# intel/neural-speed

Measured on NVIDIA H100. Metric: decode tokens/s + prefill tok/s Llama-2-7B Q4_0 @1 GPU; % HBM roofline, higher is better.
Workload: dtype int8xint4->f32 (q8_0 x q4_0)

## Files before the change

### neural_speed_b200/csrc/gemm_tc.cu

```cuda
#include <cuda.h>

#include "nsb.cuh"

namespace {

constexpr int BLOCK_N = 128;
constexpr int BLOCK_K = 64;
constexpr int WG_K = 16;
constexpr int DEQ_TILE = BLOCK_N * BLOCK_K * 2;
constexpr int kConsumerThreads = 256, kDequantThreads = 128, kThreads = kConsumerThreads + kDequantThreads + 32;

struct GemmParams {
  const uint8_t* rows;
  int wfmt, f4kind;
  int pitch, sc_off, zp_off, stype, asym, group, ngroups;
  int n, k, kpad, m;
  float* dst;
  int ldo;
  const float* bias;
  int bias_bcast;
  const float* residual;
  int kb_per_split;
  int dbg;
};

__device__ __forceinline__ uint32_t smem_u32(const void* p) { return (uint32_t)__cvta_generic_to_shared(p); }
__device__ __forceinline__ void mbar_init(uint64_t* bar, int count) {
  asm volatile("mbarrier.init.shared::cta.b64 [%0], %1;" ::"r"(smem_u32(bar)), "r"(count) : "memory");
}
__device__ __forceinline__ void mbar_expect_tx(uint64_t* bar, uint32_t bytes) {
  asm volatile("mbarrier.arrive.expect_tx.shared::cta.b64 _, [%0], %1;" ::"r"(smem_u32(bar)), "r"(bytes) : "memory");
}
__device__ __forceinline__ void mbar_arrive(uint64_t* bar) {
  asm volatile("mbarrier.arrive.shared::cta.b64 _, [%0];" ::"r"(smem_u32(bar)) : "memory");
}
__device__ __forceinline__ void mbar_wait(uint64_t* bar, uint32_t parity) {
  uint32_t ok;
  do {
    asm volatile(
        "{\n"
        ".reg .pred p;\n"
        "mbarrier.try_wait.parity.shared::cta.b64 p, [%1], %2;\n"
        "selp.u32 %0, 1, 0, p;\n"
        "}\n"
        : "=r"(ok)
        : "r"(smem_u32(bar)), "r"(parity)
        : "memory");
  } while (!ok);
}
__device__ __forceinline__ void tma_load_2d(void* dst, const CUtensorMap* map, int x, int y, uint64_t* bar) {
  asm volatile(
      "cp.async.bulk.tensor.2d.shared::cluster.global.tile.mbarrier::complete_tx::bytes [%0], [%1, {%2, %3}], [%4];" ::"r"(
          smem_u32(dst)),
      "l"(map), "r"(x), "r"(y), "r"(smem_u32(bar))
      : "memory");
}
__device__ __forceinline__ uint64_t make_desc_sw128(uint32_t smem_addr) {
  return (uint64_t)((smem_addr & 0x3FFFFu) >> 4) | (1ull << 16) | (64ull << 32) | (1ull << 62);
}
__device__ __forceinline__ void wgmma_fence() { asm volatile("wgmma.fence.sync.aligned;" ::: "memory"); }
__device__ __forceinline__ void wgmma_commit() { asm volatile("wgmma.commit_group.sync.aligned;" ::: "memory"); }
template <int N>
__device__ __forceinline__ void wgmma_wait() {
  asm volatile("wgmma.wait_group.sync.aligned %0;" ::"n"(N) : "memory");
}
__device__ __forceinline__ void wgmma_m64n32k16(float (&d)[16], uint64_t adesc, uint64_t bdesc) {
  asm volatile(
      "{\n.reg .pred p;\nsetp.ne.b32 p, %18, 0;\n"
      "wgmma.mma_async.sync.aligned.m64n32k16.f32.bf16.bf16 {"
      "%0, %1, %2, %3, %4, %5, %6, %7, %8, %9, %10, %11, %12, %13, %14, %15"
      "}, %16, %17, p, 1, 1, 0, 0;\n}\n"
      : "+f"(d[0]), "+f"(d[1]), "+f"(d[2]), "+f"(d[3]), "+f"(d[4]), "+f"(d[5]), "+f"(d[6]), "+f"(d[7]),
        "+f"(d[8]), "+f"(d[9]), "+f"(d[10]), "+f"(d[11]), "+f"(d[12]), "+f"(d[13]), "+f"(d[14]), "+f"(d[15])
      : "l"(adesc), "l"(bdesc), "r"(1));
}
__device__ __forceinline__ void wgmma_m64n64k16(float (&d)[32], uint64_t adesc, uint64_t bdesc) {
  asm volatile(
      "{\n.reg .pred p;\nsetp.ne.b32 p, %34, 0;\n"
      "wgmma.mma_async.sync.aligned.m64n64k16.f32.bf16.bf16 {"
      "%0, %1, %2, %3, %4, %5, %6, %7, %8, %9, %10, %11, %12, %13, %14, %15, "
      "%16, %17, %18, %19, %20, %21, %22, %23, %24, %25, %26, %27, %28, %29, %30, %31"
      "}, %32, %33, p, 1, 1, 0, 0;\n}\n"
      : "+f"(d[0]), "+f"(d[1]), "+f"(d[2]), "+f"(d[3]), "+f"(d[4]), "+f"(d[5]), "+f"(d[6]), "+f"(d[7]),
        "+f"(d[8]), "+f"(d[9]), "+f"(d[10]), "+f"(d[11]), "+f"(d[12]), "+f"(d[13]), "+f"(d[14]), "+f"(d[15]),
        "+f"(d[16]), "+f"(d[17]), "+f"(d[18]), "+f"(d[19]), "+f"(d[20]), "+f"(d[21]), "+f"(d[22]), "+f"(d[23]),
        "+f"(d[24]), "+f"(d[25]), "+f"(d[26]), "+f"(d[27]), "+f"(d[28]), "+f"(d[29]), "+f"(d[30]), "+f"(d[31])
      : "l"(adesc), "l"(bdesc), "r"(1));
}
__device__ __forceinline__ void wgmma_m64n128k16(float (&d)[64], uint64_t adesc, uint64_t bdesc) {
  asm volatile(
      "{\n.reg .pred p;\nsetp.ne.b32 p, %66, 0;\n"
      "wgmma.mma_async.sync.aligned.m64n128k16.f32.bf16.bf16 {"
      "%0, %1, %2, %3, %4, %5, %6, %7, %8, %9, %10, %11, %12, %13, %14, %15, "
      "%16, %17, %18, %19, %20, %21, %22, %23, %24, %25, %26, %27, %28, %29, %30, %31, "
      "%32, %33, %34, %35, %36, %37, %38, %39, %40, %41, %42, %43, %44, %45, %46, %47, "
      "%48, %49, %50, %51, %52, %53, %54, %55, %56, %57, %58, %59, %60, %61, %62, %63"
      "}, %64, %65, p, 1, 1, 0, 0;\n}\n"
      : "+f"(d[0]), "+f"(d[1]), "+f"(d[2]), "+f"(d[3]), "+f"(d[4]), "+f"(d[5]), "+f"(d[6]), "+f"(d[7]),
        "+f"(d[8]), "+f"(d[9]), "+f"(d[10]), "+f"(d[11]), "+f"(d[12]), "+f"(d[13]), "+f"(d[14]), "+f"(d[15]),
        "+f"(d[16]), "+f"(d[17]), "+f"(d[18]), "+f"(d[19]), "+f"(d[20]), "+f"(d[21]), "+f"(d[22]), "+f"(d[23]),
        "+f"(d[24]), "+f"(d[25]), "+f"(d[26]), "+f"(d[27]), "+f"(d[28]), "+f"(d[29]), "+f"(d[30]), "+f"(d[31]),
        "+f"(d[32]), "+f"(d[33]), "+f"(d[34]), "+f"(d[35]), "+f"(d[36]), "+f"(d[37]), "+f"(d[38]), "+f"(d[39]),
        "+f"(d[40]), "+f"(d[41]), "+f"(d[42]), "+f"(d[43]), "+f"(d[44]), "+f"(d[45]), "+f"(d[46]), "+f"(d[47]),
        "+f"(d[48]), "+f"(d[49]), "+f"(d[50]), "+f"(d[51]), "+f"(d[52]), "+f"(d[53]), "+f"(d[54]), "+f"(d[55]),
        "+f"(d[56]), "+f"(d[57]), "+f"(d[58]), "+f"(d[59]), "+f"(d[60]), "+f"(d[61]), "+f"(d[62]), "+f"(d[63])
      : "l"(adesc), "l"(bdesc), "r"(1));
}

template <int T>
__device__ __forceinline__ void wgmma_k16(float (&d)[T / 2], uint64_t adesc, uint64_t bdesc) {
  if constexpr (T == 32) wgmma_m64n32k16(d, adesc, bdesc);
  else if constexpr (T == 64) wgmma_m64n64k16(d, adesc, bdesc);
  else wgmma_m64n128k16(d, adesc, bdesc);
}

template <int T, bool W8 = false>
struct Smem {
  static constexpr int SP = 6;
  static constexpr int SD = 3;
  static constexpr int SA = T >= 128 ? 4 : 6;
  static constexpr int ROW_BYTES = W8 ? BLOCK_K : BLOCK_K / 2;
  static constexpr int PACKED_STAGE = BLOCK_N * ROW_BYTES;
  static constexpr int DEQ_STAGE = DEQ_TILE;
  static constexpr int ACT_STAGE = T * BLOCK_K * 2;
  static constexpr int off_deq = 0;
  static constexpr int off_act = off_deq + SD * DEQ_STAGE;
  static constexpr int off_packed = off_act + SA * ACT_STAGE;
  static constexpr int off_bar = off_packed + SP * PACKED_STAGE;
  static constexpr int num_bars = 2 * SP + 2 * SA + 2 * SD;
  static constexpr int total = off_bar + num_bars * 8 + 1024;
};

template <int T, bool W8>
__global__ void __launch_bounds__(kThreads, 1)
    gemm_w4_tc_kernel(const __grid_constant__ CUtensorMap tmap_w, const __grid_constant__ CUtensorMap tmap_a, const GemmParams P) {
  using L = Smem<T, W8>;
  constexpr int ROW_BYTES = L::ROW_BYTES;
  constexpr int SA = L::SA, SP = L::SP, SD = L::SD, PACKED_STAGE = L::PACKED_STAGE, DEQ_STAGE = L::DEQ_STAGE;
  extern __shared__ unsigned char smem_raw[];
  unsigned char* smem = smem_raw + ((1024 - (smem_u32(smem_raw) & 1023)) & 1023);
  unsigned char* deq = smem + L::off_deq;
  unsigned char* act = smem + L::off_act;
  unsigned char* packed = smem + L::off_packed;
  uint64_t* bars = reinterpret_cast<uint64_t*>(smem + L::off_bar);
  uint64_t* p_full = bars;
  uint64_t* p_empty = p_full + SP;
  uint64_t* a_full = p_empty + SP;
  uint64_t* a_empty = a_full + SA;
  uint64_t* d_full = a_empty + SA;
  uint64_t* d_empty = d_full + SD;

  const int warp = threadIdx.x >> 5, lane = threadIdx.x & 31;
  const int n0 = blockIdx.x * BLOCK_N;
  const int t0 = blockIdx.y * T;
  const int total_kb = (P.kpad + BLOCK_K - 1) / BLOCK_K;
  const int kb0 = blockIdx.z * P.kb_per_split;
  const int num_kb = (total_kb - kb0 < P.kb_per_split) ? total_kb - kb0 : P.kb_per_split;

  __shared__ float nf4_lut[16];
  if (threadIdx.x >= 32 && threadIdx.x < 48) nf4_lut[threadIdx.x - 32] = NS_F4_LUT[P.f4kind][threadIdx.x - 32];
  pdl_launch_dependents();
  if (threadIdx.x == 0) {
    for (int i = 0; i < SP; ++i) {
      mbar_init(&p_full[i], 1);
      mbar_init(&p_empty[i], kDequantThreads / 32);
    }
    for (int i = 0; i < SA; ++i) {
      mbar_init(&a_full[i], 1);
      mbar_init(&a_empty[i], kConsumerThreads / 128);
    }
    for (int i = 0; i < SD; ++i) {
      mbar_init(&d_full[i], kDequantThreads / 32);
      mbar_init(&d_empty[i], kConsumerThreads / 128);
    }
    asm volatile("fence.mbarrier_init.release.cluster;" ::: "memory");
  }
  if (warp == 12 && lane == 0) {
    asm volatile("prefetch.tensormap [%0];" ::"l"(&tmap_w) : "memory");
    asm volatile("prefetch.tensormap [%0];" ::"l"(&tmap_a) : "memory");
  }
  __syncthreads();

  if (warp == 12) {
    if (lane == 0) {
      const int pre = num_kb < SP ? num_kb : SP;
      for (int kb = 0; kb < pre; ++kb) {
        mbar_expect_tx(&p_full[kb], PACKED_STAGE);
        tma_load_2d(packed + kb * PACKED_STAGE, &tmap_w, (kb0 + kb) * ROW_BYTES, n0, &p_full[kb]);
      }
      pdl_wait();
      for (int kb = 0; kb < num_kb; ++kb) {
        const int sa = kb % SA;
        if (kb >= SA) mbar_wait(&a_empty[sa], ((kb / SA) - 1) & 1);
        mbar_expect_tx(&a_full[sa], L::ACT_STAGE);
        tma_load_2d(act + sa * L::ACT_STAGE, &tmap_a, (kb0 + kb) * BLOCK_K, t0, &a_full[sa]);
        const int kp = kb + SP;
        if (kp < num_kb) {
          const int sp = kp % SP;
          mbar_wait(&p_empty[sp], ((kp / SP) - 1) & 1);
          mbar_expect_tx(&p_full[sp], PACKED_STAGE);
          tma_load_2d(packed + sp * PACKED_STAGE, &tmap_w, (kb0 + kp) * ROW_BYTES, n0, &p_full[sp]);
        }
      }
    }
  } else if (warp >= 8) {
    const int r = threadIdx.x - kConsumerThreads;
    int grow = n0 + r;
    if (grow >= P.n) grow = P.n - 1;
    const uint8_t* rowp = P.rows + (size_t)grow * P.pitch;
    const int swz = r & 7;
    for (int kb = 0; kb < num_kb; ++kb) {
      const int sp = kb % SP, sd = kb % SD;
      int g0 = ((kb0 + kb) * BLOCK_K) / P.group, g1 = ((kb0 + kb) * BLOCK_K + 32) / P.group;
      if (g0 >= P.ngroups) g0 = P.ngroups - 1;
      if (g1 >= P.ngroups) g1 = P.ngroups - 1;
      const float sc0 = ns_scale_at(rowp + P.sc_off, P.stype, g0);
      const float sc1 = (g1 == g0) ? sc0 : ns_scale_at(rowp + P.sc_off, P.stype, g1);
      float of0 = W8 ? 0.f : 136.f, of1 = of0;
      if (P.asym) {
        of0 += (float)(int)(signed char)rowp[P.zp_off + g0];
        of1 += (float)(int)(signed char)rowp[P.zp_off + g1];
      }
      const __nv_bfloat162 s2[2] = {__float2bfloat162_rn(sc0), __float2bfloat162_rn(sc1)};
      const __nv_bfloat162 o2[2] = {__float2bfloat162_rn(of0), __float2bfloat162_rn(of1)};

      mbar_wait(&p_full[sp], (kb / SP) & 1);
      const uint4* pk = reinterpret_cast<const uint4*>(packed + sp * PACKED_STAGE + r * ROW_BYTES);
      uint32_t words[W8 ? 16 : 8];
#pragma unroll
      for (int i = 0; i < (W8 ? 4 : 2); ++i) {
        const uint4 qv = pk[i];
        words[4 * i] = qv.x, words[4 * i + 1] = qv.y, words[4 * i + 2] = qv.z, words[4 * i + 3] = qv.w;
      }
      __syncwarp();
      if (lane == 0) mbar_arrive(&p_empty[sp]);
      if (kb >= SD) mbar_wait(&d_empty[sd], ((kb / SD) - 1) & 1);
      unsigned char* drow_base = deq + sd * DEQ_STAGE + (r >> 3) * 1024 + swz * 128;
      if (!(P.dbg & 1))
#pragma unroll
      for (int c = 0; c < 8; ++c) {
        const int h = c >> 2;
        uint32_t o[4];
        if (W8) {
#pragma unroll
          for (int j = 0; j < 4; ++j) {
            const uint32_t wsrc = words[2 * c + (j >> 1)];
            const int b0 = (int)(signed char)((wsrc >> (16 * (j & 1))) & 0xffu), b1 = (int)(signed char)((wsrc >> (16 * (j & 1) + 8)) & 0xffu);
            __nv_bfloat162 v = __floats2bfloat162_rn((float)b0, (float)b1);
            v = __hmul2(__hsub2(v, o2[h]), s2[h]);
            o[j] = *reinterpret_cast<uint32_t*>(&v);
          }
        } else if (P.wfmt == NS_W_NF4) {
#pragma unroll
          for (int j = 0; j < 4; ++j) {
            const float l0 = nf4_lut[(words[c] >> (4 * j)) & 0xFu], l1 = nf4_lut[(words[c] >> (4 * j + 16)) & 0xFu];
            __nv_bfloat162 v = __hmul2(__floats2bfloat162_rn(l0, l1), s2[h]);
            o[j] = *reinterpret_cast<uint32_t*>(&v);
          }
        } else {
#pragma unroll
          for (int j = 0; j < 4; ++j) {
            uint32_t t = ((words[c] >> (4 * j)) & 0x000F000Fu) | 0x43004300u;
            __nv_bfloat162 v = *reinterpret_cast<__nv_bfloat162*>(&t);
            v = __hmul2(__hsub2(v, o2[h]), s2[h]);
            o[j] = *reinterpret_cast<uint32_t*>(&v);
          }
        }
        *reinterpret_cast<uint4*>(drow_base + ((c ^ swz) << 4)) = make_uint4(o[0], o[1], o[2], o[3]);
      }
      asm volatile("fence.proxy.async.shared::cta;" ::: "memory");
      __syncwarp();
      if (lane == 0) mbar_arrive(&d_full[sd]);
    }
  } else {
    const int g = warp >> 2;
    const bool leader = (threadIdx.x & 127) == 0;
    float acc[T / 2];
#pragma unroll
    for (int i = 0; i < T / 2; ++i) acc[i] = 0.f;
    for (int kb = 0; kb < num_kb; ++kb) {
      const int sd = kb % SD, sa = kb % SA;
      mbar_wait(&d_full[sd], (kb / SD) & 1);
      mbar_wait(&a_full[sa], (kb / SA) & 1);
      const uint32_t a_addr = smem_u32(deq + sd * DEQ_STAGE) + g * (64 * BLOCK_K * 2);
      const uint32_t b_addr = smem_u32(act + sa * L::ACT_STAGE);
      if (!(P.dbg & 2)) {
        wgmma_fence();
#pragma unroll
        for (int k4 = 0; k4 < BLOCK_K / WG_K; ++k4)
          wgmma_k16<T>(acc, make_desc_sw128(a_addr + k4 * WG_K * 2), make_desc_sw128(b_addr + k4 * WG_K * 2));
        wgmma_commit();
      }
      wgmma_wait<1>();
      if (kb > 0 && leader) {
        mbar_arrive(&d_empty[(kb - 1) % SD]);
        mbar_arrive(&a_empty[(kb - 1) % SA]);
      }
    }
    wgmma_wait<0>();
    pdl_wait();
    if (!(P.dbg & 4)) {
#pragma unroll
      for (int h = 0; h < 2; ++h) {
        const int nrow = n0 + g * 64 + (warp & 3) * 16 + (lane >> 2) + 8 * h;
        if (nrow >= P.n) continue;
        const float bcast_bias = (P.bias && P.bias_bcast) ? P.bias[nrow] : 0.f;
#pragma unroll
        for (int j = 0; j < T / 8; ++j)
#pragma unroll
          for (int e = 0; e < 2; ++e) {
            const int t = t0 + 8 * j + 2 * (lane & 3) + e;
            if (t < P.m) {
              const size_t o = (size_t)t * P.ldo + nrow;
              float x = acc[4 * j + 2 * h + e];
              if (blockIdx.z == 0) {
                x += bcast_bias;
                if (P.bias && !P.bias_bcast) x += P.bias[o];
                if (P.residual) x += P.residual[o];
              }
              if (gridDim.z > 1) atomicAdd(P.dst + o, x);
              else P.dst[o] = x;
            }
          }
      }
    }
  }
}

__global__ void __launch_bounds__(256) act_to_bf16_kernel(const float* __restrict__ A, int lda, int M, int K, int kpad,
                                                          const int* __restrict__ shuffle, __nv_bfloat16* __restrict__ out) {
  pdl_launch_dependents();
  pdl_wait();
  const size_t idx = (size_t)blockIdx.x * blockDim.x + threadIdx.x;
  const size_t total = (size_t)M * (kpad >> 1);
  if (idx >= total) return;
  const int m = (int)(idx / (kpad >> 1)), k = (int)(idx - (size_t)m * (kpad >> 1)) * 2;
  float a = 0.f, b = 0.f;
  if (k < K) a = A[(size_t)m * lda + (shuffle ? shuffle[k] : k)];
  if (k + 1 < K) b = A[(size_t)m * lda + (shuffle ? shuffle[k + 1] : k + 1)];
  reinterpret_cast<__nv_bfloat162*>(out)[idx] = __floats2bfloat162_rn(a, b);
}
__global__ void __launch_bounds__(256) act_to_bf16_v8_kernel(const float* __restrict__ A, int lda, int M, int K,
                                                             __nv_bfloat16* __restrict__ out) {
  pdl_launch_dependents();
  pdl_wait();
  const int k8 = K >> 3;
  const size_t total = (size_t)M * k8;
  for (size_t idx = (size_t)blockIdx.x * blockDim.x + threadIdx.x; idx < total; idx += (size_t)gridDim.x * blockDim.x) {
    const int m = (int)(idx / k8), c = (int)(idx - (size_t)m * k8);
    const float4* src = (const float4*)(A + (size_t)m * lda) + 2 * c;
    const float4 x = src[0], y = src[1];
    __nv_bfloat162 p0 = __floats2bfloat162_rn(x.x, x.y), p1 = __floats2bfloat162_rn(x.z, x.w);
    __nv_bfloat162 p2 = __floats2bfloat162_rn(y.x, y.y), p3 = __floats2bfloat162_rn(y.z, y.w);
    uint4 o;
    o.x = *(uint32_t*)&p0, o.y = *(uint32_t*)&p1, o.z = *(uint32_t*)&p2, o.w = *(uint32_t*)&p3;
    ((uint4*)out)[idx] = o;
  }
}

typedef CUresult (*EncodeTiledFn)(CUtensorMap*, CUtensorMapDataType, cuuint32_t, void*, const cuuint64_t*, const cuuint64_t*,
                                  const cuuint32_t*, const cuuint32_t*, CUtensorMapInterleave, CUtensorMapSwizzle,
                                  CUtensorMapL2promotion, CUtensorMapFloatOOBfill);
EncodeTiledFn get_encode() {
  static EncodeTiledFn fn = nullptr;
  if (!fn) {
    void* p = nullptr;
    cudaDriverEntryPointQueryResult qres;
    if (cudaGetDriverEntryPoint("cuTensorMapEncodeTiled", &p, cudaEnableDefault, &qres) == cudaSuccess &&
        qres == cudaDriverEntryPointSuccess)
      fn = (EncodeTiledFn)p;
  }
  return fn;
}

template <int T, bool W8>
int launch_t(const CUtensorMap& mw, const CUtensorMap& ma, const GemmParams& P, cudaStream_t st) {
  using L = Smem<T, W8>;
  auto kern = gemm_w4_tc_kernel<T, W8>;
  static bool attr_set = false;
  if (!attr_set) {
    NS_CUDA_TRY(cudaFuncSetAttribute(kern, cudaFuncAttributeMaxDynamicSharedMemorySize, L::total));
    attr_set = true;
  }
  dim3 grid((P.n + BLOCK_N - 1) / BLOCK_N, (P.m + T - 1) / T);
  GemmParams Q = P;
  const int total_kb = (P.kpad + BLOCK_K - 1) / BLOCK_K;
  int splits = 1;
  const int tiles = (int)(grid.x * grid.y);
  static const int env_splits = getenv("NS_TC_SPLITS") ? atoi(getenv("NS_TC_SPLITS")) : 0;
  if (3 * tiles < 2 * ns_num_sms() && P.residual != P.dst && P.bias != P.dst) {
    splits = ns_num_sms() / tiles;
    if (splits > total_kb / 8) splits = total_kb / 8;
    if (splits > 16) splits = 16;
    if (splits < 1) splits = 1;
  }
  if (env_splits > 0) splits = env_splits;
  Q.kb_per_split = (total_kb + splits - 1) / splits;
  splits = (total_kb + Q.kb_per_split - 1) / Q.kb_per_split;
  grid.z = (unsigned)splits;
  if (splits > 1) NS_CUDA_TRY(cudaMemset2DAsync(P.dst, (size_t)P.ldo * 4, 0, (size_t)P.n * 4, (size_t)P.m, st));
  NS_CUDA_TRY(ns_launch_pdl(kern, grid, dim3(kThreads), (size_t)L::total, st, mw, ma, Q));
  ns_count_launch();
  return NS_OK;
}

}

size_t ns_gemm_tc_workspace_bytes(int m, int kpad) { return ns_round_up((size_t)m * kpad * 2, 256); }

bool ns_gemm_tc_supported(const ns_weight* w) {
  return (w->wfmt == NS_W_S4 || w->wfmt == NS_W_NF4 || w->wfmt == NS_W_S8) && (w->group % 32 == 0 || w->group == w->k);
}

int ns_launch_act_bf16(const ns_weight* w, const float* act, int lda, int m, void* ws, cudaStream_t st) {
  if (!w->shuffle && w->k == w->kpad && (w->k & 7) == 0 && (lda & 3) == 0 && ((uintptr_t)act & 15) == 0) {
    const size_t total8 = (size_t)m * (w->k >> 3);
    size_t blocks = (total8 + 255) / 256;
    if (blocks > (size_t)ns_num_sms() * 16) blocks = (size_t)ns_num_sms() * 16;
    NS_CUDA_TRY(ns_launch_pdl(act_to_bf16_v8_kernel, dim3((unsigned)blocks), dim3(256), 0, st, act, lda, m, w->k, (__nv_bfloat16*)ws));
    ns_count_launch();
    return NS_OK;
  }
  const size_t total = (size_t)m * (w->kpad >> 1);
  NS_CUDA_TRY(ns_launch_pdl(act_to_bf16_kernel, dim3((unsigned)((total + 255) / 256)), dim3(256), 0, st, act, lda, m, w->k,
                            w->kpad, (const int*)w->shuffle, (__nv_bfloat16*)ws));
  ns_count_launch();
  return NS_OK;
}

template <bool V4>
__global__ void __launch_bounds__(256) silu_mul_kernel(const float* __restrict__ g, const float* __restrict__ u,
// ... 90 lines not shown
  }
  const __nv_bfloat16* abf = (const __nv_bfloat16*)ws;
  const int T = m <= 32 ? 32 : (m <= 64 ? 64 : 128);
  const bool w8 = w->wfmt == NS_W_S8;
  CUtensorMap mw, ma;
  {
    cuuint64_t dims[2] = {(cuuint64_t)w->q_bytes, (cuuint64_t)w->n};
    cuuint64_t strides[1] = {(cuuint64_t)w->pitch};
    cuuint32_t box[2] = {(cuuint32_t)(w8 ? BLOCK_K : BLOCK_K / 2), (cuuint32_t)BLOCK_N};
    cuuint32_t es[2] = {1, 1};
    CUresult r = enc(&mw, CU_TENSOR_MAP_DATA_TYPE_UINT8, 2, (void*)w->rows, dims, strides, box, es, CU_TENSOR_MAP_INTERLEAVE_NONE,
                     CU_TENSOR_MAP_SWIZZLE_NONE, CU_TENSOR_MAP_L2_PROMOTION_L2_128B, CU_TENSOR_MAP_FLOAT_OOB_FILL_NONE);
    if (r != CUDA_SUCCESS) {
      ns_set_error("cuTensorMapEncodeTiled(weights) failed: %d", (int)r);
      return NS_E_CUDA;
    }
  }
  {
    cuuint64_t dims[2] = {(cuuint64_t)w->kpad, (cuuint64_t)m};
    cuuint64_t strides[1] = {(cuuint64_t)w->kpad * 2};
    cuuint32_t box[2] = {BLOCK_K, (cuuint32_t)T};
    cuuint32_t es[2] = {1, 1};
    CUresult r = enc(&ma, CU_TENSOR_MAP_DATA_TYPE_BFLOAT16, 2, (void*)abf, dims, strides, box, es, CU_TENSOR_MAP_INTERLEAVE_NONE,
                     CU_TENSOR_MAP_SWIZZLE_128B, CU_TENSOR_MAP_L2_PROMOTION_L2_128B, CU_TENSOR_MAP_FLOAT_OOB_FILL_NONE);
    if (r != CUDA_SUCCESS) {
      ns_set_error("cuTensorMapEncodeTiled(activations) failed: %d", (int)r);
      return NS_E_CUDA;
    }
  }
  GemmParams P;
  P.rows = w->rows;
  P.wfmt = w->wfmt;
  P.f4kind = w->f4kind;
  P.pitch = w->pitch;
  P.sc_off = w->sc_off;
  P.zp_off = w->zp_off;
  P.stype = w->stype;
  P.asym = w->asym;
  P.group = w->group;
  P.ngroups = w->ngroups;
  P.n = w->n;
  P.k = w->k;
  P.kpad = w->kpad;
  P.m = m;
  P.dst = dst;
  P.ldo = ldo;
  P.bias = bias;
  P.bias_bcast = bias_bcast;
  P.residual = residual;
  static const int dbg = getenv("NS_TC_DEBUG") ? atoi(getenv("NS_TC_DEBUG")) : 0;
  P.dbg = dbg;
  if (w8) {
    switch (T) {
      case 32: return launch_t<32, true>(mw, ma, P, st);
      case 64: return launch_t<64, true>(mw, ma, P, st);
      default: return launch_t<128, true>(mw, ma, P, st);
    }
  }
  switch (T) {
    case 32: return launch_t<32, false>(mw, ma, P, st);
    case 64: return launch_t<64, false>(mw, ma, P, st);
    default: return launch_t<128, false>(mw, ma, P, st);
  }
}
```

### neural_speed_b200/csrc/gemv_ring_impl.cuh

```cuda
#pragma once
#include "act_quant.cuh"

namespace {

constexpr int kConsumers = 7;
constexpr int kThreads = (kConsumers + 1) * 32;

__device__ __forceinline__ uint32_t smem_u32(const void* p) { return (uint32_t)__cvta_generic_to_shared(p); }
__device__ __forceinline__ void mbar_init(uint32_t bar, int count) {
  asm volatile("mbarrier.init.shared::cta.b64 [%0], %1;" ::"r"(bar), "r"(count) : "memory");
}
__device__ __forceinline__ void mbar_expect_tx(uint32_t bar, uint32_t bytes) {
  asm volatile("mbarrier.arrive.expect_tx.shared::cta.b64 _, [%0], %1;" ::"r"(bar), "r"(bytes) : "memory");
}
__device__ __forceinline__ void mbar_arrive(uint32_t bar) {
  asm volatile("mbarrier.arrive.shared::cta.b64 _, [%0];" ::"r"(bar) : "memory");
}
__device__ __forceinline__ void mbar_wait(uint32_t bar, uint32_t parity) {
  uint32_t ok;
  do {
    asm volatile(
        "{\n"
        ".reg .pred p;\n"
        "mbarrier.try_wait.parity.shared::cta.b64 p, [%1], %2;\n"
// ... 432 lines not shown
            const float g = acc[0][m], up = acc[ROWS - 1][m];
            const float sg = P.eltop == NS_ELT_GELU ? ns_gelu(g) : ns_silu(g);
            if (P.aux) P.aux[(size_t)m * P.ldo + ps.out0] = sg;
            P.dst[(size_t)m * P.ldo + ps.out0] = sg * up;
          }
        }
      } else {
#pragma unroll
        for (int r = 0; r < ROWS; ++r) {
          if (r == 1 && !ps.valid1) continue;
          const long long out = r ? ps.out1 : ps.out0;
#pragma unroll
          for (int m = 0; m < M; ++m) {
            if (m < P.m) {
              const size_t o = (size_t)m * P.ldo + out;
              float v = acc[r][m];
              if (P.bias) v += P.bias_bcast ? P.bias[out] : P.bias[o];
              if (P.eltop == NS_ELT_GELU) v = ns_gelu(v);
              if (P.residual) v += P.residual[o];
              P.dst[o] = v;
            }
          }
        }
      }
    }
  }
}

struct RingPlan {
  int rows, stages, active, ctas;
  size_t budget;
  double score;
};

static RingPlan plan_ring(const GemvParams& P, size_t act_region, bool wide) {
  static const int env_budget = getenv("NS_RING_BUDGET_KB") ? atoi(getenv("NS_RING_BUDGET_KB")) : 0;
  static const int env_rows = getenv("NS_RING_ROWS") ? atoi(getenv("NS_RING_ROWS")) : 0;
  const size_t budgets[2] = {(size_t)(env_budget > 0 ? env_budget : 113) * 1024, 200 * 1024};
  RingPlan best = {0, 0, 0, 0, 0, -1.0};
  for (int rows = 2; rows >= 1; --rows) {
    if (rows == 1 && P.mode == NS_GEMV_GATE_UP_SILU) continue;
    if (env_rows && rows != env_rows && !(env_rows == 1 && P.mode == NS_GEMV_GATE_UP_SILU)) continue;
    const int stage_bytes = rows * P.pitch;
    for (int i = 0; i < 2; ++i) {
      if (wide && i == 0) continue;
      const int kc = (wide && i == 1) ? 2 * kConsumers : kConsumers;
      int raw = 0;
      if (budgets[i] > act_region + 64) raw = (int)((budgets[i] - act_region - 64) / (stage_bytes + 16));
      if (raw > (wide ? 56 : 32)) raw = wide ? 56 : 32;
      const int ac = raw < kc ? raw : kc;
      if (ac < 1) continue;
      const int st = raw - raw % ac;
      const int ctas = i == 0 ? 2 : 1;
      const double score = ctas * ac * (rows == 2 ? 1.1 : 1.0) + 0.001 * st;
      if (score > best.score) best = RingPlan{rows, st, ac, ctas, budgets[i], score};
    }
  }
  return best;
}

template <int AMODE, int M, bool ASYM, int STYPE, int ROWS, bool NORM, int NC = kConsumers>
int launch_rows(const GemvParams& P, const RingPlan& plan, size_t act_region, int act_row, int red_off, cudaStream_t st) {
  auto kern = gemv_ring_kernel<AMODE, M, ASYM, STYPE, ROWS, NORM, NC>;
  constexpr int threads = (NC + (NC > kConsumers ? 2 : 1)) * 32;
  static bool attr_set = false;
  if (!attr_set) {
    NS_CUDA_TRY(cudaFuncSetAttribute(kern, cudaFuncAttributeMaxDynamicSharedMemorySize, 200 * 1024));
    attr_set = true;
  }
  const int stage_bytes = ROWS * P.pitch;
  const size_t smem = act_region + (size_t)plan.stages * stage_bytes + (size_t)plan.stages * 16;
  static const int env_cps = getenv("NS_RING_CPS") ? atoi(getenv("NS_RING_CPS")) : 0;
  const int ctas_per_sm = plan.ctas == 1 ? 1 : (env_cps > 0 ? env_cps : 2);
  RingCfg R;
  R.ring_off = (int)act_region;
  R.stages = plan.stages;
  R.active = plan.active;
  R.act_row = act_row;
  R.red_off = red_off;
  if (ROWS == 2) {
    R.units = P.npairs;
  } else {
    long long rows = 0;
    for (int i = 0; i < P.nw; ++i) rows += P.n[i];
    R.units = (int)rows;
  }
  R.cpg_magic = P.cpg > 1 ? (uint32_t)((0x100000000ull + (uint64_t)P.cpg - 1) / (uint64_t)P.cpg) : 0u;
  int grid = ns_num_sms() * ctas_per_sm;
  if (grid > R.units) grid = R.units;
  if (grid < 1) grid = 1;
  static const bool dbg = getenv("NS_RING_DEBUG") != nullptr;
  if (dbg)
    fprintf(stderr, "gemv_ring: k=%d pitch=%d rows/stage=%d stages=%d active=%d smem=%zu ctas/sm=%d\n", P.k, P.pitch, ROWS, plan.stages,
            plan.active, smem, ctas_per_sm);
  NS_CUDA_TRY(ns_launch_pdl(kern, dim3(grid), dim3(threads), smem, st, P, R));
  ns_count_launch();
  return NS_OK;
}

}
```

Before: 646.0.

## Dequantize weights in consumer registers and feed wgmma A from registers

Restructures the prefill tensor-core GEMM. The dedicated dequant warpgroup and the dequantized shared-memory tile are removed. Consumer warps now read packed int4/int8 weights from shared memory, dequantize them in registers, and issue register-sourced wgmma with BLOCK_N raised to 256. Producer warps prefetch per-stage scales and offsets, setmaxnreg rebalances registers, and the epilogue stages output through shared memory for coalesced stores. Separately, the GEMV ring planner adds a wave-balance factor to its score, and a prefill A/B benchmark script is added. Risks include register pressure in consumers and dequant ALU work now sitting on the MMA critical path.

```diff
diff --git a/neural_speed_b200/csrc/gemm_tc.cu b/neural_speed_b200/csrc/gemm_tc.cu
--- a/neural_speed_b200/csrc/gemm_tc.cu
+++ b/neural_speed_b200/csrc/gemm_tc.cu
@@ -4,11 +4,12 @@
 
 namespace {
 
-constexpr int BLOCK_N = 128;
+constexpr int BLOCK_N = 256;
 constexpr int BLOCK_K = 64;
 constexpr int WG_K = 16;
-constexpr int DEQ_TILE = BLOCK_N * BLOCK_K * 2;
-constexpr int kConsumerThreads = 256, kDequantThreads = 128, kThreads = kConsumerThreads + kDequantThreads + 32;
+constexpr int kConsumerThreads = 256, kThreads = kConsumerThreads + 128;
+constexpr int kScaleThreads = 64;
+constexpr int kProducerRegs = 56, kConsumerRegs = 224;
 
 struct GemmParams {
   const uint8_t* rows;
@@ -64,38 +65,38 @@
 __device__ __forceinline__ void wgmma_wait() {
   asm volatile("wgmma.wait_group.sync.aligned %0;" ::"n"(N) : "memory");
 }
-__device__ __forceinline__ void wgmma_m64n32k16(float (&d)[16], uint64_t adesc, uint64_t bdesc) {
+__device__ __forceinline__ void wgmma_m64n32k16(float (&d)[16], const uint32_t (&a)[4], uint64_t bdesc) {
   asm volatile(
-      "{\n.reg .pred p;\nsetp.ne.b32 p, %18, 0;\n"
+      "{\n.reg .pred p;\nsetp.ne.b32 p, %21, 0;\n"
       "wgmma.mma_async.sync.aligned.m64n32k16.f32.bf16.bf16 {"
       "%0, %1, %2, %3, %4, %5, %6, %7, %8, %9, %10, %11, %12, %13, %14, %15"
-      "}, %16, %17, p, 1, 1, 0, 0;\n}\n"
+      "}, {%16, %17, %18, %19}, %20, p, 1, 1, 0;\n}\n"
       : "+f"(d[0]), "+f"(d[1]), "+f"(d[2]), "+f"(d[3]), "+f"(d[4]), "+f"(d[5]), "+f"(d[6]), "+f"(d[7]),
         "+f"(d[8]), "+f"(d[9]), "+f"(d[10]), "+f"(d[11]), "+f"(d[12]), "+f"(d[13]), "+f"(d[14]), "+f"(d[15])
-      : "l"(adesc), "l"(bdesc), "r"(1));
-}
-__device__ __forceinline__ void wgmma_m64n64k16(float (&d)[32], uint64_t adesc, uint64_t bdesc) {
+      : "r"(a[0]), "r"(a[1]), "r"(a[2]), "r"(a[3]), "l"(bdesc), "r"(1));
+}
+__device__ __forceinline__ void wgmma_m64n64k16(float (&d)[32], const uint32_t (&a)[4], uint64_t bdesc) {
   asm volatile(
-      "{\n.reg .pred p;\nsetp.ne.b32 p, %34, 0;\n"
+      "{\n.reg .pred p;\nsetp.ne.b32 p, %37, 0;\n"
       "wgmma.mma_async.sync.aligned.m64n64k16.f32.bf16.bf16 {"
       "%0, %1, %2, %3, %4, %5, %6, %7, %8, %9, %10, %11, %12, %13, %14, %15, "
       "%16, %17, %18, %19, %20, %21, %22, %23, %24, %25, %26, %27, %28, %29, %30, %31"
-      "}, %32, %33, p, 1, 1, 0, 0;\n}\n"
+      "}, {%32, %33, %34, %35}, %36, p, 1, 1, 0;\n}\n"
       : "+f"(d[0]), "+f"(d[1]), "+f"(d[2]), "+f"(d[3]), "+f"(d[4]), "+f"(d[5]), "+f"(d[6]), "+f"(d[7]),
         "+f"(d[8]), "+f"(d[9]), "+f"(d[10]), "+f"(d[11]), "+f"(d[12]), "+f"(d[13]), "+f"(d[14]), "+f"(d[15]),
         "+f"(d[16]), "+f"(d[17]), "+f"(d[18]), "+f"(d[19]), "+f"(d[20]), "+f"(d[21]), "+f"(d[22]), "+f"(d[23]),
         "+f"(d[24]), "+f"(d[25]), "+f"(d[26]), "+f"(d[27]), "+f"(d[28]), "+f"(d[29]), "+f"(d[30]), "+f"(d[31])
-      : "l"(adesc), "l"(bdesc), "r"(1));
-}
-__device__ __forceinline__ void wgmma_m64n128k16(float (&d)[64], uint64_t adesc, uint64_t bdesc) {
+      : "r"(a[0]), "r"(a[1]), "r"(a[2]), "r"(a[3]), "l"(bdesc), "r"(1));
+}
+__device__ __forceinline__ void wgmma_m64n128k16(float (&d)[64], const uint32_t (&a)[4], uint64_t bdesc) {
   asm volatile(
-      "{\n.reg .pred p;\nsetp.ne.b32 p, %66, 0;\n"
+      "{\n.reg .pred p;\nsetp.ne.b32 p, %69, 0;\n"
       "wgmma.mma_async.sync.aligned.m64n128k16.f32.bf16.bf16 {"
       "%0, %1, %2, %3, %4, %5, %6, %7, %8, %9, %10, %11, %12, %13, %14, %15, "
       "%16, %17, %18, %19, %20, %21, %22, %23, %24, %25, %26, %27, %28, %29, %30, %31, "
       "%32, %33, %34, %35, %36, %37, %38, %39, %40, %41, %42, %43, %44, %45, %46, %47, "
       "%48, %49, %50, %51, %52, %53, %54, %55, %56, %57, %58, %59, %60, %61, %62, %63"
-      "}, %64, %65, p, 1, 1, 0, 0;\n}\n"
+      "}, {%64, %65, %66, %67}, %68, p, 1, 1, 0;\n}\n"
       : "+f"(d[0]), "+f"(d[1]), "+f"(d[2]), "+f"(d[3]), "+f"(d[4]), "+f"(d[5]), "+f"(d[6]), "+f"(d[7]),
         "+f"(d[8]), "+f"(d[9]), "+f"(d[10]), "+f"(d[11]), "+f"(d[12]), "+f"(d[13]), "+f"(d[14]), "+f"(d[15]),
         "+f"(d[16]), "+f"(d[17]), "+f"(d[18]), "+f"(d[19]), "+f"(d[20]), "+f"(d[21]), "+f"(d[22]), "+f"(d[23]),
@@ -104,51 +105,66 @@
         "+f"(d[40]), "+f"(d[41]), "+f"(d[42]), "+f"(d[43]), "+f"(d[44]), "+f"(d[45]), "+f"(d[46]), "+f"(d[47]),
         "+f"(d[48]), "+f"(d[49]), "+f"(d[50]), "+f"(d[51]), "+f"(d[52]), "+f"(d[53]), "+f"(d[54]), "+f"(d[55]),
         "+f"(d[56]), "+f"(d[57]), "+f"(d[58]), "+f"(d[59]), "+f"(d[60]), "+f"(d[61]), "+f"(d[62]), "+f"(d[63])
-      : "l"(adesc), "l"(bdesc), "r"(1));
+      : "r"(a[0]), "r"(a[1]), "r"(a[2]), "r"(a[3]), "l"(bdesc), "r"(1));
 }
 
 template <int T>
-__device__ __forceinline__ void wgmma_k16(float (&d)[T / 2], uint64_t adesc, uint64_t bdesc) {
-  if constexpr (T == 32) wgmma_m64n32k16(d, adesc, bdesc);
-  else if constexpr (T == 64) wgmma_m64n64k16(d, adesc, bdesc);
-  else wgmma_m64n128k16(d, adesc, bdesc);
-}
-
-template <int T, bool W8 = false>
+__device__ __forceinline__ void wgmma_k16(float (&d)[T / 2], const uint32_t (&a)[4], uint64_t bdesc) {
+  if constexpr (T == 32) wgmma_m64n32k16(d, a, bdesc);
+  else if constexpr (T == 64) wgmma_m64n64k16(d, a, bdesc);
+  else wgmma_m64n128k16(d, a, bdesc);
+}
+
+template <int T, int WFMT>
 struct Smem {
   static constexpr int SP = 6;
-  static constexpr int SD = 3;
-  static constexpr int SA = T >= 128 ? 4 : 6;
-  static constexpr int ROW_BYTES = W8 ? BLOCK_K : BLOCK_K / 2;
+  static constexpr int SA = T >= 128 ? 5 : 6;
+  static constexpr int ROW_BYTES = WFMT == NS_W_S8 ? BLOCK_K : BLOCK_K / 2;
   static constexpr int PACKED_STAGE = BLOCK_N * ROW_BYTES;
-  static constexpr int DEQ_STAGE = DEQ_TILE;
+  static constexpr int SCALE_STAGE = BLOCK_N * 16;
   static constexpr int ACT_STAGE = T * BLOCK_K * 2;
-  static constexpr int off_deq = 0;
-  static constexpr int off_act = off_deq + SD * DEQ_STAGE;
+  static constexpr int off_act = 0;
   static constexpr int off_packed = off_act + SA * ACT_STAGE;
-  static constexpr int off_bar = off_packed + SP * PACKED_STAGE;
-  static constexpr int num_bars = 2 * SP + 2 * SA + 2 * SD;
+  static constexpr int off_scale = off_packed + SP * PACKED_STAGE;
+  static constexpr int off_bar = off_scale + SP * SCALE_STAGE;
+  static constexpr int num_bars = 2 * SP + 2 * SA;
   static constexpr int total = off_bar + num_bars * 8 + 1024;
 };
 
-template <int T, bool W8>
+template <int WFMT>
+__device__ __forceinline__ uint32_t dequant_pair(uint32_t w, int c, uint32_t s, uint32_t o, const float* lut) {
+  __nv_bfloat162 v;
+  if constexpr (WFMT == NS_W_S8) {
+    const int sh = 16 * (c & 1);
+    v = __floats2bfloat162_rn((float)(int)(signed char)((w >> sh) & 0xffu), (float)(int)(signed char)((w >> (sh + 8)) & 0xffu));
+    v = __hsub2(v, *reinterpret_cast<const __nv_bfloat162*>(&o));
+  } else if constexpr (WFMT == NS_W_NF4) {
+    v = __floats2bfloat162_rn(lut[(w >> (4 * c)) & 0xFu], lut[(w >> (4 * c + 16)) & 0xFu]);
+  } else {
+    uint32_t t = ((w >> (4 * c)) & 0x000F000Fu) | 0x43004300u;
+    v = __hsub2(*reinterpret_cast<__nv_bfloat162*>(&t), *reinterpret_cast<const __nv_bfloat162*>(&o));
+  }
+  v = __hmul2(v, *reinterpret_cast<const __nv_bfloat162*>(&s));
+  return *reinterpret_cast<uint32_t*>(&v);
+}
+
+template <int T, int WFMT>
 __global__ void __launch_bounds__(kThreads, 1)
     gemm_w4_tc_kernel(const __grid_constant__ CUtensorMap tmap_w, const __grid_constant__ CUtensorMap tmap_a, const GemmParams P) {
-  using L = Smem<T, W8>;
+  using L = Smem<T, WFMT>;
+  constexpr bool W8 = WFMT == NS_W_S8;
   constexpr int ROW_BYTES = L::ROW_BYTES;
-  constexpr int SA = L::SA, SP = L::SP, SD = L::SD, PACKED_STAGE = L::PACKED_STAGE, DEQ_STAGE = L::DEQ_STAGE;
+  constexpr int SA = L::SA, SP = L::SP, PACKED_STAGE = L::PACKED_STAGE, SCALE_STAGE = L::SCALE_STAGE;
   extern __shared__ unsigned char smem_raw[];
   unsigned char* smem = smem_raw + ((1024 - (smem_u32(smem_raw) & 1023)) & 1023);
-  unsigned char* deq = smem + L::off_deq;
   unsigned char* act = smem + L::off_act;
   unsigned char* packed = smem + L::off_packed;
+  unsigned char* scales = smem + L::off_scale;
   uint64_t* bars = reinterpret_cast<uint64_t*>(smem + L::off_bar);
   uint64_t* p_full = bars;
   uint64_t* p_empty = p_full + SP;
   uint64_t* a_full = p_empty + SP;
   uint64_t* a_empty = a_full + SA;
-  uint64_t* d_full = a_empty + SA;
-  uint64_t* d_empty = d_full + SD;
 
   const int warp = threadIdx.x >> 5, lane = threadIdx.x & 31;
   const int n0 = blockIdx.x * BLOCK_N;
@@ -162,27 +178,25 @@
   pdl_launch_dependents();
   if (threadIdx.x == 0) {
     for (int i = 0; i < SP; ++i) {
-      mbar_init(&p_full[i], 1);
-      mbar_init(&p_empty[i], kDequantThreads / 32);
+      mbar_init(&p_full[i], 1 + kScaleThreads);
+      mbar_init(&p_empty[i], kConsumerThreads / 32);
     }
     for (int i = 0; i < SA; ++i) {
       mbar_init(&a_full[i], 1);
-      mbar_init(&a_empty[i], kConsumerThreads / 128);
-    }
-    for (int i = 0; i < SD; ++i) {
-      mbar_init(&d_full[i], kDequantThreads / 32);
-      mbar_init(&d_empty[i], kConsumerThreads / 128);
+      mbar_init(&a_empty[i], kConsumerThreads / 32);
     }
     asm volatile("fence.mbarrier_init.release.cluster;" ::: "memory");
   }
-  if (warp == 12 && lane == 0) {
+  if (threadIdx.x == kConsumerThreads) {
     asm volatile("prefetch.tensormap [%0];" ::"l"(&tmap_w) : "memory");
     asm volatile("prefetch.tensormap [%0];" ::"l"(&tmap_a) : "memory");
   }
   __syncthreads();
 
-  if (warp == 12) {
-    if (lane == 0) {
+  if (threadIdx.x >= kConsumerThreads) {
+    asm volatile("setmaxnreg.dec.sync.aligned.u32 %0;" ::"n"(kProducerRegs));
+    const int pwarp = warp - kConsumerThreads / 32;
+    if (pwarp == 0 && lane == 0) {
       const int pre = num_kb < SP ? num_kb : SP;
       for (int kb = 0; kb < pre; ++kb) {
         mbar_expect_tx(&p_full[kb], PACKED_STAGE);
@@ -202,126 +216,125 @@
           tma_load_2d(packed + sp * PACKED_STAGE, &tmap_w, (kb0 + kp) * ROW_BYTES, n0, &p_full[sp]);
         }
       }
-    }
-  } else if (warp >= 8) {
-    const int r = threadIdx.x - kConsumerThreads;
-    int grow = n0 + r;
-    if (grow >= P.n) grow = P.n - 1;
-    const uint8_t* rowp = P.rows + (size_t)grow * P.pitch;
-    const int swz = r & 7;
+    } else if (pwarp == 1 || pwarp == 2) {
+      const int i = threadIdx.x - kConsumerThreads - 32;
+      const uint8_t* rowp[4];
+#pragma unroll
+      for (int j = 0; j < 4; ++j) {
+        int grow = n0 + i + 64 * j;
+        if (grow >= P.n) grow = P.n - 1;
+        rowp[j] = P.rows + (size_t)grow * P.pitch;
+      }
+      for (int kb = 0; kb < num_kb; ++kb) {
+        const int sp = kb % SP;
+        int g0 = ((kb0 + kb) * BLOCK_K) / P.group, g1 = ((kb0 + kb) * BLOCK_K + 32) / P.group;
+        if (g0 >= P.ngroups) g0 = P.ngroups - 1;
+        if (g1 >= P.ngroups) g1 = P.ngroups - 1;
+        uint4 v[4];
+#pragma unroll
+        for (int j = 0; j < 4; ++j) {
+          const float sc0 = ns_scale_at(rowp[j] + P.sc_off, P.stype, g0);
+          const float sc1 = (g1 == g0) ? sc0 : ns_scale_at(rowp[j] + P.sc_off, P.stype, g1);
+          float of0 = W8 ? 0.f : 136.f, of1 = of0;
+          if (P.asym) {
+            of0 += (float)(int)(signed char)rowp[j][P.zp_off + g0];
+            of1 += (float)(int)(signed char)rowp[j][P.zp_off + g1];
+          }
+          __nv_bfloat162 s0 = __float2bfloat162_rn(sc0), s1 = __float2bfloat162_rn(sc1);
+          __nv_bfloat162 o0 = __float2bfloat162_rn(of0), o1 = __float2bfloat162_rn(of1);
+          v[j] = make_uint4(*reinterpret_cast<uint32_t*>(&s0), *reinterpret_cast<uint32_t*>(&s1), *reinterpret_cast<uint32_t*>(&o0),
+                            *reinterpret_cast<uint32_t*>(&o1));
+        }
+        if (kb >= SP) mbar_wait(&p_empty[sp], ((kb / SP) - 1) & 1);
+#pragma unroll
+        for (int j = 0; j < 4; ++j) reinterpret_cast<uint4*>(scales + sp * SCALE_STAGE)[i + 64 * j] = v[j];
+        mbar_arrive(&p_full[sp]);
+      }
+    }
+  } else {
+    asm volatile("setmaxnreg.inc.sync.aligned.u32 %0;" ::"n"(kConsumerRegs));
+    const int g = warp >> 2, c = lane & 3;
+    const int rbase = 128 * g + 16 * (warp & 3) + (lane >> 2);
+    const bool deq = !(P.dbg & 1), mma = !(P.dbg & 2);
+    float acc[2][T / 2];
+#pragma unroll
+    for (int h = 0; h < 2; ++h)
+#pragma unroll
+      for (int i = 0; i < T / 2; ++i) acc[h][i] = 0.f;
     for (int kb = 0; kb < num_kb; ++kb) {
-      const int sp = kb % SP, sd = kb % SD;
-      int g0 = ((kb0 + kb) * BLOCK_K) / P.group, g1 = ((kb0 + kb) * BLOCK_K + 32) / P.group;
-      if (g0 >= P.ngroups) g0 = P.ngroups - 1;
-      if (g1 >= P.ngroups) g1 = P.ngroups - 1;
-      const float sc0 = ns_scale_at(rowp + P.sc_off, P.stype, g0);
-      const float sc1 = (g1 == g0) ? sc0 : ns_scale_at(rowp + P.sc_off, P.stype, g1);
-      float of0 = W8 ? 0.f : 136.f, of1 = of0;
-      if (P.asym) {
-        of0 += (float)(int)(signed char)rowp[P.zp_off + g0];
-        of1 += (float)(int)(signed char)rowp[P.zp_off + g1];
-      }
-      const __nv_bfloat162 s2[2] = {__float2bfloat162_rn(sc0), __float2bfloat162_rn(sc1)};
-      const __nv_bfloat162 o2[2] = {__float2bfloat162_rn(of0), __float2bfloat162_rn(of1)};
-
+      const int sp = kb % SP, sa = kb % SA;
       mbar_wait(&p_full[sp], (kb / SP) & 1);
-      const uint4* pk = reinterpret_cast<const uint4*>(packed + sp * PACKED_STAGE + r * ROW_BYTES);
-      uint32_t words[W8 ? 16 : 8];
-#pragma unroll
-      for (int i = 0; i < (W8 ? 4 : 2); ++i) {
-        const uint4 qv = pk[i];
-        words[4 * i] = qv.x, words[4 * i + 1] = qv.y, words[4 * i + 2] = qv.z, words[4 * i + 3] = qv.w;
-      }
-      __syncwarp();
-      if (lane == 0) mbar_arrive(&p_empty[sp]);
-      if (kb >= SD) mbar_wait(&d_empty[sd], ((kb / SD) - 1) & 1);
-      unsigned char* drow_base = deq + sd * DEQ_STAGE + (r >> 3) * 1024 + swz * 128;
-      if (!(P.dbg & 1))
-#pragma unroll
-      for (int c = 0; c < 8; ++c) {
-        const int h = c >> 2;
-        uint32_t o[4];
-        if (W8) {
-#pragma unroll
-          for (int j = 0; j < 4; ++j) {
-            const uint32_t wsrc = words[2 * c + (j >> 1)];
-            const int b0 = (int)(signed char)((wsrc >> (16 * (j & 1))) & 0xffu), b1 = (int)(signed char)((wsrc >> (16 * (j & 1) + 8)) & 0xffu);
-            __nv_bfloat162 v = __floats2bfloat162_rn((float)b0, (float)b1);
-            v = __hmul2(__hsub2(v, o2[h]), s2[h]);
-            o[j] = *reinterpret_cast<uint32_t*>(&v);
-          }
-        } else if (P.wfmt == NS_W_NF4) {
-#pragma unroll
-          for (int j = 0; j < 4; ++j) {
-            const float l0 = nf4_lut[(words[c] >> (4 * j)) & 0xFu], l1 = nf4_lut[(words[c] >> (4 * j + 16)) & 0xFu];
-            __nv_bfloat162 v = __hmul2(__floats2bfloat162_rn(l0, l1), s2[h]);
-            o[j] = *reinterpret_cast<uint32_t*>(&v);
-          }
+      uint32_t raw[4][8];
+      uint4 sc[4];
+#pragma unroll
+      for (int r = 0; r < 4; ++r) {
+        const int row = rbase + 64 * (r >> 1) + 8 * (r & 1);
+        const unsigned char* src = packed + sp * PACKED_STAGE + row * ROW_BYTES;
+        if constexpr (W8) {
+#pragma unroll
+          for (int i = 0; i < 8; ++i) raw[r][i] = reinterpret_cast<const uint32_t*>(src)[2 * i + (c >> 1)];
         } else {
-#pragma unroll
-          for (int j = 0; j < 4; ++j) {
-            uint32_t t = ((words[c] >> (4 * j)) & 0x000F000Fu) | 0x43004300u;
-            __nv_bfloat162 v = *reinterpret_cast<__nv_bfloat162*>(&t);
-            v = __hmul2(__hsub2(v, o2[h]), s2[h]);
-            o[j] = *reinterpret_cast<uint32_t*>(&v);
-          }
+          const uint4 q0 = reinterpret_cast<const uint4*>(src)[0], q1 = reinterpret_cast<const uint4*>(src)[1];
+          raw[r][0] = q0.x, raw[r][1] = q0.y, raw[r][2] = q0.z, raw[r][3] = q0.w;
+          raw[r][4] = q1.x, raw[r][5] = q1.y, raw[r][6] = q1.z, raw[r][7] = q1.w;
         }
-        *reinterpret_cast<uint4*>(drow_base + ((c ^ swz) << 4)) = make_uint4(o[0], o[1], o[2], o[3]);
+        sc[r] = reinterpret_cast<const uint4*>(scales + sp * SCALE_STAGE)[row];
       }
       asm volatile("fence.proxy.async.shared::cta;" ::: "memory");
       __syncwarp();
-      if (lane == 0) mbar_arrive(&d_full[sd]);
-    }
-  } else {
-    const int g = warp >> 2;
-    const bool leader = (threadIdx.x & 127) == 0;
-    float acc[T / 2];
-#pragma unroll
-    for (int i = 0; i < T / 2; ++i) acc[i] = 0.f;
-    for (int kb = 0; kb < num_kb; ++kb) {
-      const int sd = kb % SD, sa = kb % SA;
-      mbar_wait(&d_full[sd], (kb / SD) & 1);
+      if (lane == 0) mbar_arrive(&p_empty[sp]);
       mbar_wait(&a_full[sa], (kb / SA) & 1);
-      const uint32_t a_addr = smem_u32(deq + sd * DEQ_STAGE) + g * (64 * BLOCK_K * 2);
       const uint32_t b_addr = smem_u32(act + sa * L::ACT_STAGE);
-      if (!(P.dbg & 2)) {
-        wgmma_fence();
-#pragma unroll
-        for (int k4 = 0; k4 < BLOCK_K / WG_K; ++k4)
-          wgmma_k16<T>(acc, make_desc_sw128(a_addr + k4 * WG_K * 2), make_desc_sw128(b_addr + k4 * WG_K * 2));
-        wgmma_commit();
-      }
-      wgmma_wait<1>();
-      if (kb > 0 && leader) {
-        mbar_arrive(&d_empty[(kb - 1) % SD]);
-        mbar_arrive(&a_empty[(kb - 1) % SA]);
+#pragma unroll
+      for (int s = 0; s < BLOCK_K / WG_K; ++s) {
+        uint32_t a[2][4];
+#pragma unroll
+        for (int hf = 0; hf < 2; ++hf)
+#pragma unroll
+          for (int j = 0; j < 4; ++j) {
+            const int r = 2 * hf + (j & 1);
+            const uint32_t w = raw[r][2 * s + (j >> 1)];
+            a[hf][j] = deq ? dequant_pair<WFMT>(w, c, s < 2 ? sc[r].x : sc[r].y, s < 2 ? sc[r].z : sc[r].w, nf4_lut) : (w | 0x43004300u);
+          }
+        if (mma) {
+          wgmma_fence();
+          wgmma_k16<T>(acc[0], a[0], make_desc_sw128(b_addr + s * WG_K * 2));
+          wgmma_k16<T>(acc[1], a[1], make_desc_sw128(b_addr + s * WG_K * 2));
+          wgmma_commit();
+        }
+        wgmma_wait<1>();
+        if (s == 0 && kb > 0 && lane == 0) mbar_arrive(&a_empty[(kb - 1) % SA]);
       }
     }
     wgmma_wait<0>();
     pdl_wait();
     if (!(P.dbg & 4)) {
-#pragma unroll
-      for (int h = 0; h < 2; ++h) {
-        const int nrow = n0 + g * 64 + (warp & 3) * 16 + (lane >> 2) + 8 * h;
-        if (nrow >= P.n) continue;
-        const float bcast_bias = (P.bias && P.bias_bcast) ? P.bias[nrow] : 0.f;
+      constexpr int EP = BLOCK_N + 4;
+      static_assert(T * EP * 4 <= L::off_bar, "epilogue tile must fit below the barriers");
+      float* tile = reinterpret_cast<float*>(smem);
+      asm volatile("bar.sync 1, %0;" ::"n"(kConsumerThreads) : "memory");
+#pragma unroll
+      for (int hf = 0; hf < 2; ++hf)
 #pragma unroll
         for (int j = 0; j < T / 8; ++j)
 #pragma unroll
-          for (int e = 0; e < 2; ++e) {
-            const int t = t0 + 8 * j + 2 * (lane & 3) + e;
-            if (t < P.m) {
-              const size_t o = (size_t)t * P.ldo + nrow;
-              float x = acc[4 * j + 2 * h + e];
-              if (blockIdx.z == 0) {
-                x += bcast_bias;
-                if (P.bias && !P.bias_bcast) x += P.bias[o];
-                if (P.residual) x += P.residual[o];
-              }
-              if (gridDim.z > 1) atomicAdd(P.dst + o, x);
-              else P.dst[o] = x;
-            }
-          }
+          for (int h = 0; h < 2; ++h)
+#pragma unroll
+            for (int e = 0; e < 2; ++e) tile[(8 * j + 2 * c + e) * EP + rbase + 64 * hf + 8 * h] = acc[hf][4 * j + 2 * h + e];
+      asm volatile("bar.sync 1, %0;" ::"n"(kConsumerThreads) : "memory");
+      const bool split0 = blockIdx.z == 0, atomic = gridDim.z > 1;
+      for (int i = threadIdx.x; i < T * BLOCK_N; i += kConsumerThreads) {
+        const int t = t0 + i / BLOCK_N, nrow = n0 + i % BLOCK_N;
+        if (t >= P.m || nrow >= P.n) continue;
+        const size_t o = (size_t)t * P.ldo + nrow;
+        float x = tile[(i / BLOCK_N) * EP + i % BLOCK_N];
+        if (split0) {
+          x += (P.bias && P.bias_bcast) ? P.bias[nrow] : 0.f;
+          if (P.bias && !P.bias_bcast) x += P.bias[o];
+          if (P.residual) x += P.residual[o];
+        }
+        if (atomic) atomicAdd(P.dst + o, x);
+        else P.dst[o] = x;
       }
     }
   }
@@ -373,10 +386,10 @@
   return fn;
 }
 
-template <int T, bool W8>
+template <int T, int WFMT>
 int launch_t(const CUtensorMap& mw, const CUtensorMap& ma, const GemmParams& P, cudaStream_t st) {
-  using L = Smem<T, W8>;
-  auto kern = gemm_w4_tc_kernel<T, W8>;
+  using L = Smem<T, WFMT>;
+  auto kern = gemm_w4_tc_kernel<T, WFMT>;
   static bool attr_set = false;
   if (!attr_set) {
     NS_CUDA_TRY(cudaFuncSetAttribute(kern, cudaFuncAttributeMaxDynamicSharedMemorySize, L::total));
@@ -573,14 +586,21 @@
   P.dbg = dbg;
   if (w8) {
     switch (T) {
-      case 32: return launch_t<32, true>(mw, ma, P, st);
-      case 64: return launch_t<64, true>(mw, ma, P, st);
-      default: return launch_t<128, true>(mw, ma, P, st);
+      case 32: return launch_t<32, NS_W_S8>(mw, ma, P, st);
+      case 64: return launch_t<64, NS_W_S8>(mw, ma, P, st);
+      default: return launch_t<128, NS_W_S8>(mw, ma, P, st);
+    }
+  }
+  if (w->wfmt == NS_W_NF4) {
+    switch (T) {
+      case 32: return launch_t<32, NS_W_NF4>(mw, ma, P, st);
+      case 64: return launch_t<64, NS_W_NF4>(mw, ma, P, st);
+      default: return launch_t<128, NS_W_NF4>(mw, ma, P, st);
     }
   }
   switch (T) {
-    case 32: return launch_t<32, false>(mw, ma, P, st);
-    case 64: return launch_t<64, false>(mw, ma, P, st);
-    default: return launch_t<128, false>(mw, ma, P, st);
-  }
-}
+    case 32: return launch_t<32, NS_W_S4>(mw, ma, P, st);
+    case 64: return launch_t<64, NS_W_S4>(mw, ma, P, st);
+    default: return launch_t<128, NS_W_S4>(mw, ma, P, st);
+  }
+}
diff --git a/neural_speed_b200/csrc/gemv_ring_impl.cuh b/neural_speed_b200/csrc/gemv_ring_impl.cuh
--- a/neural_speed_b200/csrc/gemv_ring_impl.cuh
+++ b/neural_speed_b200/csrc/gemv_ring_impl.cuh
@@ -508,7 +508,12 @@
       if (ac < 1) continue;
       const int st = raw - raw % ac;
       const int ctas = i == 0 ? 2 : 1;
-      const double score = ctas * ac * (rows == 2 ? 1.1 : 1.0) + 0.001 * st;
+      long long units = 0;
+      for (int w = 0; w < P.nw; ++w) units += P.n[w];
+      if (rows == 2) units = P.npairs;
+      const long long warps = (long long)ns_num_sms() * ctas * ac;
+      const double balance = (double)units / (double)(((units + warps - 1) / warps) * warps);
+      const double score = ctas * ac * (rows == 2 ? 1.1 : 1.0) * balance + 0.001 * st;
       if (score > best.score) best = RingPlan{rows, st, ac, ctas, budgets[i], score};
     }
   }
diff --git a/profiles/prefill_ab.py b/profiles/prefill_ab.py
--- /dev/null
+++ b/profiles/prefill_ab.py
@@ -0,0 +1,72 @@
+import argparse
+import json
+import os
+import sys
+
+ap = argparse.ArgumentParser()
+ap.add_argument("--root", required=True)
+ap.add_argument("--dump", default=None)
+ap.add_argument("--m", type=int, default=2048)
+ap.add_argument("--iters", type=int, default=20)
+args = ap.parse_args()
+sys.path.insert(0, os.path.abspath(args.root))
+
+import ctypes as C
+
+import numpy as np
+import torch
+
+import neural_speed_b200 as ns
+
+assert os.path.dirname(ns.__file__).startswith(os.path.abspath(args.root)), ns.__file__
+L = ns.lib()
+L.bestla_init()
+M, E, FF = args.m, 4096, 11008
+st = torch.cuda.Stream()
+q = C.c_void_p(st.cuda_stream)
+gen = torch.Generator(device="cuda").manual_seed(1234)
+x = torch.randn(M, FF, device="cuda", generator=gen)
+ws = torch.zeros(L.ns_device_workspace_bytes(M, FF), dtype=torch.uint8, device="cuda")
+FORMATS = {"q4_0": dict(group=32, stype=ns.S_F16, comp=ns.COMP_Q8_0), "int4_g128": dict(group=128, stype=ns.S_F32, comp=ns.COMP_INT8)}
+results = []
+if args.dump:
+    os.makedirs(args.dump, exist_ok=True)
+for fmt, kw in FORMATS.items():
+    W = {nm: ns.Weight.random(n, k, wfmt=ns.W_S4, asym=False, seed=100 + i, queue=q, **kw)
+         for i, (nm, n, k) in enumerate((("wq", E, E), ("wk", E, E), ("wv", E, E), ("wo", E, E), ("w1", FF, E), ("w3", FF, E),
+                                          ("w2", E, FF)))}
+    L.bestla_device_sync(q)
+    shapes = [("qkv", [W["wq"], W["wk"], W["wv"]], E), ("o", [W["wo"]], E), ("gate", [W["w1"]], E), ("up", [W["w3"]], E),
+              ("down", [W["w2"]], FF)]
+    for name, ws_, k in shapes:
+        n = ws_[0].n
+        out = torch.full((len(ws_), M, n), float("nan"), device="cuda")
+        xp, op, wp = C.c_void_p(x.data_ptr()), C.c_void_p(out.data_ptr()), C.c_void_p(ws.data_ptr())
+        if len(ws_) == 3:
+            call = lambda: L.ns_mul_qkv(ws_[0].h, ws_[1].h, ws_[2].h, xp, FF, op, n, M, wp, q)
+        else:
+            call = lambda: L.ns_mul_mat(ws_[0].h, xp, FF, op, n, M, None, None, 0, wp, q)
+        torch.cuda.synchronize()
+        for _ in range(3):
+            assert call() == 0, ns.last_error()
+        torch.cuda.synchronize()
+        e0, e1 = torch.cuda.Event(enable_timing=True), torch.cuda.Event(enable_timing=True)
+        e0.record(st)
+        for _ in range(args.iters):
+            call()
+        e1.record(st)
+        torch.cuda.synchronize()
+        us = e0.elapsed_time(e1) * 1e3 / args.iters
+        flops = 2.0 * M * k * sum(w.n for w in ws_)
+        results.append({"fmt": fmt, "shape": name, "m": M, "n": sum(w.n for w in ws_), "k": k, "us": us, "tflops": flops / us / 1e6})
+        if args.dump:
+            np.save(os.path.join(args.dump, f"{fmt}_{name}.npy"), out.cpu().numpy())
+    for w in W.values():
+        w.free()
+for r in results:
+    print(f"{r['fmt']:10s} {r['shape']:5s} M={r['m']} N={r['n']:5d} K={r['k']:5d}: {r['us']:8.1f} us {r['tflops']:6.1f} TFLOP/s")
+for fmt in FORMATS:
+    tot = sum(r["us"] for r in results if r["fmt"] == fmt)
+    fl = sum(2.0 * r["m"] * r["n"] * r["k"] for r in results if r["fmt"] == fmt)
+    print(f"{fmt:10s} one layer's GEMMs {tot:8.1f} us = {fl / tot / 1e6:6.1f} TFLOP/s ({M * 1e6 / (32 * tot):.0f} tok/s for 32 layers)")
+print(json.dumps({"root": args.root, "results": results}))
```

Measured after the change: 647.3, median of 6. About the same (+0.2%).
